# dmosopt/dmosopt

Hardware: NVIDIA H100
Metric: candidate-evals/sec (GP+sort+HV) pop=65536 dim=30 obj=3 (higher is better)
Workload: dtype f64 results; GP variance contraction in split-fp16 wgmma with fp32 accumulation (precision=auto: calibrated against the float64 path, 0 of 65535 rows of the last step recomputed in float64); ranks on u32 ids

## Files before the change

dmosopt_b200/csrc/common.cuh:

```cuda
#pragma once

#include <cuda_runtime.h>
#include <math.h>
#include <stdint.h>
#include <stdio.h>

#include <string>
#include <vector>

#include "../../include/dmosopt_b200.h"

struct dmo_ctx {
  int device = 0;
  cudaStream_t stream = nullptr;
  cudaMemPool_t pool = nullptr;
  cudaEvent_t ev0 = nullptr, ev1 = nullptr;
  int sm_count = 132;
  int64_t launches = 0;
  int64_t waits = 0;
  std::string err;
  void* flush_buf = nullptr;
  size_t flush_bytes = 0;
  int* dev_flag = nullptr;
  uint64_t h2d_bytes = 0, d2h_bytes = 0;
  unsigned long long* lag_host = nullptr;
  cudaEvent_t lag_ev[3] = {nullptr, nullptr, nullptr};
  static constexpr int kSide = 4;
  cudaStream_t side[kSide] = {};
  cudaEvent_t side_ev[kSide + 1] = {};
  bool profiling = false;
  struct Timer {
    std::string name;
    cudaEvent_t a, b;
  };
  std::vector<Timer> timers;
};

struct ProfileScope {
  dmo_ctx* ctx;
  int idx = -1;
  ProfileScope(dmo_ctx* c, const char* name) : ctx(c) {
    if (!c->profiling) return;
    dmo_ctx::Timer t;
    t.name = name;
    if (cudaEventCreate(&t.a) != cudaSuccess || cudaEventCreate(&t.b) != cudaSuccess) return;
    cudaEventRecord(t.a, c->stream);
    c->timers.push_back(t);
    idx = (int)c->timers.size() - 1;
  }
  ~ProfileScope() {
    if (idx >= 0) cudaEventRecord(ctx->timers[idx].b, ctx->stream);
  }
};

int dmo_fail(dmo_ctx* ctx, int code, const char* fmt, ...);

#define DMO_CUDA(call)                                                                        \
  do {                                                                                        \
    cudaError_t e__ = (call);                                                                 \
    if (e__ != cudaSuccess)                                                                   \
      return dmo_fail(ctx, DMO_ERR_CUDA, "%s failed: %s (%s:%d)", #call, cudaGetErrorString(e__), \
                      __FILE__, __LINE__);                                                    \
  } while (0)

#define DMO_TRY(expr)              \
  do {                             \
    int s__ = (expr);              \
    if (s__ != DMO_OK) return s__; \
  } while (0)

#define DMO_REQUIRE(cond, ...)                                 \
  do {                                                         \
    if (!(cond)) return dmo_fail(ctx, DMO_ERR_ARG, __VA_ARGS__); \
  } while (0)

#define DMO_LAUNCH(kernel, grid, block, smem, ...)                       \
  do {                                                                   \
    kernel<<<(grid), (block), (smem), ctx->stream>>>(__VA_ARGS__);       \
    ctx->launches++;                                                     \
  } while (0)

#define DMO_CHECK_LAUNCH() DMO_CUDA(cudaGetLastError())

struct SideStreams {
  dmo_ctx* ctx;
  cudaStream_t main;
  int k = 0;
  int rc = DMO_OK;
  SideStreams(dmo_ctx* c, int nside);
  ~SideStreams();
  void on(int s) { ctx->stream = ctx->side[s]; }
  void back() { ctx->stream = main; }
};

int dmo_lag_slots(dmo_ctx* ctx);

static inline cudaError_t dmo_wait(dmo_ctx* ctx) {
  ctx->waits++;
  return cudaStreamSynchronize(ctx->stream);
}

static inline int64_t ceil_div(int64_t a, int64_t b) { return (a + b - 1) / b; }

template <typename T>
struct DevBuf {
  dmo_ctx* ctx = nullptr;
  T* p = nullptr;
  size_t n = 0;
  DevBuf() {}
  DevBuf(const DevBuf&) = delete;
  DevBuf& operator=(const DevBuf&) = delete;
  ~DevBuf() { release(); }
  int alloc(dmo_ctx* c, size_t count) {
    release();
    ctx = c;
    n = count;
    if (count == 0) count = 1;
    cudaError_t e = cudaMallocAsync((void**)&p, count * sizeof(T), c->stream);
    if (e != cudaSuccess) {
      p = nullptr;
      return dmo_fail(c, DMO_ERR_CUDA, "cudaMallocAsync(%zu bytes) failed: %s", count * sizeof(T),
                      cudaGetErrorString(e));
    }
    return DMO_OK;
  }
  void release() {
    if (p) cudaFreeAsync(p, ctx->stream);
    p = nullptr;
  }
};

bool dmo_is_device_ptr(const void* p);

template <typename T>
struct In {
  DevBuf<T> buf;
  const T* d = nullptr;
  int init(dmo_ctx* ctx, const T* src, size_t count) {
    if (src == nullptr || count == 0) {
      d = nullptr;
      return DMO_OK;
    }
    if (dmo_is_device_ptr(src)) {
      d = src;
      return DMO_OK;
    }
    DMO_TRY(buf.alloc(ctx, count));
    DMO_CUDA(cudaMemcpyAsync(buf.p, src, count * sizeof(T), cudaMemcpyHostToDevice, ctx->stream));
    ctx->h2d_bytes += count * sizeof(T);
    d = buf.p;
    return DMO_OK;
  }
};

template <typename T>
struct Out {
  DevBuf<T> buf;
  T* d = nullptr;
  T* host = nullptr;
  size_t count = 0;
  int init(dmo_ctx* ctx, T* dst, size_t cnt) {
    count = cnt;
    if (dst == nullptr) {
      d = nullptr;
      return DMO_OK;
    }
    if (dmo_is_device_ptr(dst)) {
      d = dst;
      return DMO_OK;
    }
    host = dst;
    DMO_TRY(buf.alloc(ctx, cnt));
    d = buf.p;
    return DMO_OK;
  }
  int finish(dmo_ctx* ctx, size_t cnt = (size_t)-1) {
    if (host && d) {
      size_t c = (cnt == (size_t)-1) ? count : cnt;
// ... 118 lines not shown
```

dmosopt_b200/csrc/ctx.cu:

```cuda
#include <stdarg.h>

#include "common.cuh"

int dmo_fail(dmo_ctx* ctx, int code, const char* fmt, ...) {
  char buf[1024];
  va_list ap;
  va_start(ap, fmt);
  vsnprintf(buf, sizeof(buf), fmt, ap);
  va_end(ap);
  if (ctx) ctx->err = buf;
  return code;
}

bool dmo_is_device_ptr(const void* p) {
  cudaPointerAttributes a;
  cudaError_t e = cudaPointerGetAttributes(&a, p);
  if (e != cudaSuccess) {
    cudaGetLastError();
    return false;
  }
  return a.type == cudaMemoryTypeDevice || a.type == cudaMemoryTypeManaged;
}

int dmo_lag_slots(dmo_ctx* ctx) {
  if (ctx->lag_host) return DMO_OK;
  DMO_CUDA(cudaHostAlloc((void**)&ctx->lag_host, 3 * sizeof(unsigned long long), cudaHostAllocDefault));
  for (cudaEvent_t& e : ctx->lag_ev) DMO_CUDA(cudaEventCreateWithFlags(&e, cudaEventDisableTiming));
  return DMO_OK;
}

SideStreams::SideStreams(dmo_ctx* c, int nside) : ctx(c), main(c->stream) {
  if (nside > dmo_ctx::kSide) nside = dmo_ctx::kSide;
  if (!ctx->side[0]) {
    for (cudaStream_t& st : ctx->side)
      if (cudaStreamCreateWithFlags(&st, cudaStreamNonBlocking) != cudaSuccess) rc = DMO_ERR_CUDA;
    for (cudaEvent_t& e : ctx->side_ev)
      if (cudaEventCreateWithFlags(&e, cudaEventDisableTiming) != cudaSuccess) rc = DMO_ERR_CUDA;
  }
  if (rc == DMO_OK && cudaEventRecord(ctx->side_ev[0], main) != cudaSuccess) rc = DMO_ERR_CUDA;
  for (int s = 0; rc == DMO_OK && s < nside; ++s, ++k)
    if (cudaStreamWaitEvent(ctx->side[s], ctx->side_ev[0], 0) != cudaSuccess) rc = DMO_ERR_CUDA;
  if (rc != DMO_OK) dmo_fail(ctx, rc, "could not set up side streams");
}

SideStreams::~SideStreams() {
  ctx->stream = main;
  for (int s = 0; s < k; ++s) {
    cudaEventRecord(ctx->side_ev[1 + s], ctx->side[s]);
    cudaStreamWaitEvent(main, ctx->side_ev[1 + s], 0);
  }
}

extern "C" {

int dmo_version(void) { return 100; }

int dmo_create(int device, dmo_ctx** out) {
  if (!out) return DMO_ERR_ARG;
  *out = nullptr;
  dmo_ctx* ctx = new dmo_ctx();
  ctx->device = device;
  cudaError_t e = cudaSetDevice(device);
  if (e != cudaSuccess) {
    fprintf(stderr, "dmosopt_b200: cudaSetDevice(%d) failed: %s\n", device, cudaGetErrorString(e));
    delete ctx;
    return DMO_ERR_CUDA;
  }
  cudaDeviceProp prop;
  e = cudaGetDeviceProperties(&prop, device);
  if (e != cudaSuccess) {
    delete ctx;
    return DMO_ERR_CUDA;
  }
  ctx->sm_count = prop.multiProcessorCount;
  if (cudaStreamCreateWithFlags(&ctx->stream, cudaStreamNonBlocking) != cudaSuccess ||
      cudaEventCreate(&ctx->ev0) != cudaSuccess || cudaEventCreate(&ctx->ev1) != cudaSuccess) {
    delete ctx;
    return DMO_ERR_CUDA;
  }
  if (cudaDeviceGetDefaultMemPool(&ctx->pool, device) == cudaSuccess) {
    uint64_t thr = UINT64_MAX;
    cudaMemPoolSetAttribute(ctx->pool, cudaMemPoolAttrReleaseThreshold, &thr);
  }
  if (cudaMalloc((void**)&ctx->dev_flag, 4 * sizeof(int)) != cudaSuccess) {
    delete ctx;
    return DMO_ERR_CUDA;
  }
  cudaMemset(ctx->dev_flag, 0, 4 * sizeof(int));
  *out = ctx;
  return DMO_OK;
}

int dmo_destroy(dmo_ctx* ctx) {
  if (!ctx) return DMO_OK;
  cudaSetDevice(ctx->device);
  dmo_wait(ctx);
  if (ctx->flush_buf) cudaFree(ctx->flush_buf);
  if (ctx->dev_flag) cudaFree(ctx->dev_flag);
  if (ctx->lag_host) cudaFreeHost(ctx->lag_host);
  for (cudaEvent_t e : ctx->lag_ev)
    if (e) cudaEventDestroy(e);
  for (cudaEvent_t e : ctx->side_ev)
    if (e) cudaEventDestroy(e);
  for (cudaStream_t st : ctx->side)
    if (st) cudaStreamDestroy(st);
  cudaEventDestroy(ctx->ev0);
  cudaEventDestroy(ctx->ev1);
  cudaStreamDestroy(ctx->stream);
  delete ctx;
  return DMO_OK;
}

const char* dmo_last_error(dmo_ctx* ctx) { return ctx ? ctx->err.c_str() : "null context"; }

int dmo_synchronize(dmo_ctx* ctx) {
  DMO_CUDA(dmo_wait(ctx));
  return DMO_OK;
}

void* dmo_stream(dmo_ctx* ctx) { return (void*)ctx->stream; }
int64_t dmo_launch_count(dmo_ctx* ctx) { return ctx->launches; }
int64_t dmo_wait_count(dmo_ctx* ctx) { return ctx->waits; }
int dmo_sm_count(dmo_ctx* ctx) { return ctx->sm_count; }

int dmo_timer_begin(dmo_ctx* ctx) {
  DMO_CUDA(cudaEventRecord(ctx->ev0, ctx->stream));
  return DMO_OK;
}

int dmo_timer_end(dmo_ctx* ctx, float* ms) {
  DMO_CUDA(cudaEventRecord(ctx->ev1, ctx->stream));
  ctx->waits++;
  DMO_CUDA(cudaEventSynchronize(ctx->ev1));
  DMO_CUDA(cudaEventElapsedTime(ms, ctx->ev0, ctx->ev1));
  return DMO_OK;
}

int dmo_host_alloc(void** out, uint64_t bytes) {
  return cudaHostAlloc(out, bytes ? bytes : 1, cudaHostAllocDefault) == cudaSuccess ? DMO_OK : DMO_ERR_CUDA;
}
int dmo_host_free(void* p) { return cudaFreeHost(p) == cudaSuccess ? DMO_OK : DMO_ERR_CUDA; }

int dmo_device_alloc(dmo_ctx* ctx, void** out, uint64_t bytes) {
  if (!ctx || !out) return DMO_ERR_ARG;
  DMO_CUDA(cudaSetDevice(ctx->device));
  DMO_CUDA(cudaMallocAsync(out, bytes ? bytes : 1, ctx->stream));
  return DMO_OK;
}
int dmo_device_free(dmo_ctx* ctx, void* p) {
  if (!ctx) return DMO_ERR_ARG;
  if (!p) return DMO_OK;
  DMO_CUDA(cudaFreeAsync(p, ctx->stream));
  return DMO_OK;
}

int dmo_memcpy(dmo_ctx* ctx, void* dst, const void* src, uint64_t bytes) {
  if (!ctx) return DMO_ERR_ARG;
  if (bytes == 0) return DMO_OK;
  DMO_CUDA(cudaMemcpyAsync(dst, src, bytes, cudaMemcpyDefault, ctx->stream));
  DMO_CUDA(dmo_wait(ctx));
  const bool sd = dmo_is_device_ptr(src), dd = dmo_is_device_ptr(dst);
  if (!sd && dd) ctx->h2d_bytes += bytes;
  if (sd && !dd) ctx->d2h_bytes += bytes;
  return DMO_OK;
}

int dmo_transfer_bytes(dmo_ctx* ctx, uint64_t* h2d, uint64_t* d2h) {
  if (h2d) *h2d = ctx->h2d_bytes;
  if (d2h) *d2h = ctx->d2h_bytes;
  return DMO_OK;
}

int dmo_profile_enable(dmo_ctx* ctx, int on) {
  DMO_CUDA(dmo_wait(ctx));
  for (auto& t : ctx->timers) {
    cudaEventDestroy(t.a);
    cudaEventDestroy(t.b);
  }
  ctx->timers.clear();
  ctx->profiling = on != 0;
  return DMO_OK;
}

int dmo_profile_report(dmo_ctx* ctx, char* buf, uint64_t cap) {
  DMO_CUDA(dmo_wait(ctx));
  std::vector<std::string> names;
  std::vector<double> ms;
  std::vector<int> cnt;
// ... 48 lines not shown
```

dmosopt_b200/csrc/gp.cu:

```cuda
#include <string.h>

#include <algorithm>

#include "gp.cuh"

namespace {

constexpr int TRI_B = 128;

__global__ void tri_embed_kernel(const double* __restrict__ L, int64_t ldl, int64_t sL, int64_t N, int64_t Np,
                                 double* __restrict__ Lp) {
  int64_t t = (int64_t)blockIdx.x * blockDim.x + threadIdx.x;
  if (t >= Np * Np) return;
  L += (size_t)blockIdx.y * sL;
  Lp += (size_t)blockIdx.y * Np * Np;
  int64_t r = t / Np, c = t - r * Np;
  Lp[t] = (r < N && c < N) ? (c <= r ? L[r * ldl + c] : 0.0) : (r == c ? 1.0 : 0.0);
}

__global__ void __launch_bounds__(TRI_B) tri_diag_inverse_kernel(const double* __restrict__ Lp, int64_t Np,
                                                                 double* __restrict__ X) {
  Lp += (size_t)blockIdx.y * Np * Np;
  X += (size_t)blockIdx.y * Np * Np;
  const int64_t base = (int64_t)blockIdx.x * TRI_B;
// ... 459 lines not shown
  if (t >= n * M) return;
  const int64_t r = t / M;
  const int m = (int)(t - r * M);
  const int64_t p = idx[r];
  mean[p * M + m] = msub[t];
  var[p * M + m] = vsub[t];
}

int gp_calibrate(dmo_ctx* ctx, dmo_gp* gp) {
  if (gp->calibrated) return DMO_OK;
  const int M = gp->M, d = gp->d;
  const int P = CAL_PROBES;
  gp->auto_mean_tensor = gp->auto_var_tensor = gp->auto_mean_only = false;
  gp->cal_mean_err = gp->cal_var_err = gp->cal_mean_err_only = INFINITY;
  gp->refine_theta = 1.0;
  if (M > 16 || d > 64) {
    gp->calibrated = true;
    return DMO_OK;
  }
  DevBuf<double> xn, m64, v64, mt, vt;
  DMO_TRY(xn.alloc(ctx, (size_t)P * d));
  DMO_TRY(m64.alloc(ctx, (size_t)P * M));
  DMO_TRY(v64.alloc(ctx, (size_t)P * M));
  DMO_TRY(mt.alloc(ctx, (size_t)P * M));
  DMO_TRY(vt.alloc(ctx, (size_t)P * M));
  DMO_LAUNCH(probe_points_kernel, (unsigned)ceil_div(P, 128), 128, 0, gp->Xt.p, gp->N, d, P / 2, P, xn.p);
  DMO_CHECK_LAUNCH();
  const bool prof = ctx->profiling;
  ctx->profiling = false;
  DevBuf<double> mo;
  DMO_TRY(mo.alloc(ctx, (size_t)P * M));
  int rc = gp_predict_fp64(ctx, gp, xn.p, P, m64.p, v64.p);
  if (rc == DMO_OK) rc = gp_predict_tensor(ctx, gp, xn.p, P, mt.p, vt.p);
  if (rc == DMO_OK) rc = gp_predict_tensor(ctx, gp, xn.p, P, mo.p, nullptr);
  ctx->profiling = prof;
  if (rc != DMO_OK) return rc;
  std::vector<double> h((size_t)4 * P * M), ho((size_t)P * M);
  DMO_CUDA(cudaMemcpyAsync(ho.data(), mo.p, (size_t)P * M * 8, cudaMemcpyDeviceToHost, ctx->stream));
  DMO_CUDA(cudaMemcpyAsync(h.data(), m64.p, (size_t)P * M * 8, cudaMemcpyDeviceToHost, ctx->stream));
  DMO_CUDA(cudaMemcpyAsync(h.data() + (size_t)P * M, v64.p, (size_t)P * M * 8, cudaMemcpyDeviceToHost, ctx->stream));
  DMO_CUDA(cudaMemcpyAsync(h.data() + (size_t)2 * P * M, mt.p, (size_t)P * M * 8, cudaMemcpyDeviceToHost, ctx->stream));
  DMO_CUDA(cudaMemcpyAsync(h.data() + (size_t)3 * P * M, vt.p, (size_t)P * M * 8, cudaMemcpyDeviceToHost, ctx->stream));
  DMO_CUDA(dmo_wait(ctx));
  const double *a64 = h.data(), *b64 = a64 + (size_t)P * M, *at = b64 + (size_t)P * M, *bt = at + (size_t)P * M;
  double em = 0.0, ev = 0.0, eo = 0.0;
  for (int p = 0; p < P; ++p)
    for (int m = 0; m < M; ++m) {
      const double ys = gp->h_ystd[m];
      const double prior = (gp->h_constant[m] + gp->h_noise[m]) * ys * ys;
      const double dm = fabs(at[p * M + m] - a64[p * M + m]) / fmax(fabs(a64[p * M + m]), ys);
      const double dv = fabs(bt[p * M + m] - b64[p * M + m]) / prior;
      em = (dm > em || dm != dm) ? (dm != dm ? INFINITY : dm) : em;
      ev = (dv > ev || dv != dv) ? (dv != dv ? INFINITY : dv) : ev;
      const double dq = fabs(ho[p * M + m] - a64[p * M + m]) / fmax(fabs(a64[p * M + m]), ys);
      eo = (dq > eo || dq != dq) ? (dq != dq ? INFINITY : dq) : eo;
    }
  gp->cal_mean_err = em;
  gp->cal_mean_err_only = eo;
  gp->cal_var_err = ev;
  gp->auto_mean_tensor = em <= 2.5e-6;
  gp->auto_mean_only = eo <= 2.5e-6;
  gp->auto_var_tensor = gp->auto_mean_tensor && ev <= 4.5e-6;
  gp->refine_theta = fmax(0.02, 2.0 * ev / 1e-5);
  gp->calibrated = true;
  if (getenv("DMO_GP_VERBOSE"))
    fprintf(stderr, "dmosopt_b200: GP calibration (N=%lld d=%d M=%d): mean err K*alpha %.3e, mean-only kernel %.3e, var err/prior %.3e -> mean %s, var %s, theta %.3f\n",
            (long long)gp->N, d, M, em, eo, ev, gp->auto_mean_tensor ? "K*alpha pass" : "float64", gp->auto_var_tensor ? "tensor" : "float64", gp->refine_theta);
  return DMO_OK;
}

int gp_predict_auto(dmo_ctx* ctx, dmo_gp* gp, const double* dXn, int64_t P, double* d_mean, double* d_var,
                    GpPending* pending) {
  DMO_TRY(gp_calibrate(ctx, gp));
  gp->last_refined = 0;
  if (d_var ? !gp->auto_var_tensor : !gp->auto_mean_only) {
    gp->last_refined = P;
    return gp_predict_fp64(ctx, gp, dXn, P, d_mean, d_var);
  }
  if (!d_var) return gp_predict_tensor(ctx, gp, dXn, P, d_mean, nullptr);
  GpPending own;
  GpPending& q = pending ? *pending : own;
  DMO_TRY(q.flag.alloc(ctx, (size_t)P + 1));
  DMO_TRY(q.pos.alloc(ctx, (size_t)P + 2));
  DMO_TRY(gp_predict_tensor(ctx, gp, dXn, P, d_mean, d_var, q.pos.p + P + 1));
  DMO_CUDA(cudaMemsetAsync(q.flag.p + P, 0, sizeof(int32_t), ctx->stream));
  DMO_LAUNCH(flag_small_var_kernel, (unsigned)ceil_div(P, 256), 256, 0, d_var, P, gp->M, gp->constant.p, gp->noise.p, gp->ystd.p,
             gp->refine_theta, q.flag.p);
  DMO_TRY(prim_exclusive_sum_i32(ctx, q.flag.p, q.pos.p, P + 1));
  DMO_TRY(dmo_lag_slots(ctx));
  DMO_CUDA(cudaMemcpyAsync(ctx->lag_host + 2, q.pos.p + P, 2 * sizeof(int32_t), cudaMemcpyDeviceToHost, ctx->stream));
  DMO_CUDA(cudaEventRecord(ctx->lag_ev[2], ctx->stream));
  q.active = true;
  q.P = P;
  q.dXn = dXn;
  q.d_mean = d_mean;
  q.d_var = d_var;
  if (pending) return DMO_OK;
  bool refined = false;
  return gp_predict_finish(ctx, gp, q, &refined);
}

}

__global__ void linear_mean_add_kernel(const double* __restrict__ Xn, int64_t P, int d, int M,
                                       const double* __restrict__ w, const double* __restrict__ b,
                                       const double* __restrict__ ystd, double* __restrict__ mean) {
  const int64_t t = (int64_t)blockIdx.x * blockDim.x + threadIdx.x;
  if (t >= P * M) return;
  const int64_t p = t / M;
  const int m = (int)(t - p * M);
  double s = b[m];
  for (int j = 0; j < d; ++j) s = fma(w[m * d + j], Xn[p * d + j], s);
  mean[t] += ystd[m] * s;
}

int gp_predict_finish(dmo_ctx* ctx, dmo_gp* gp, GpPending& q, bool* refined) {
  *refined = false;
  if (!q.active) return DMO_OK;
  q.active = false;
  ctx->waits++;
  DMO_CUDA(cudaEventSynchronize(ctx->lag_ev[2]));
  int32_t h[2];
  memcpy(h, ctx->lag_host + 2, sizeof(h));
  if (h[1]) return dmo_fail(ctx, DMO_ERR_INTERNAL, "%s", GP_WATCHDOG_MSG);
  const int32_t n_ref = h[0];
  gp->last_refined = n_ref;
  if (n_ref == 0) return DMO_OK;
  const int M = gp->M, d = gp->d;
  const int64_t P = q.P;
  DevBuf<int32_t> idx;
  DevBuf<double> xs, ms, vs;
  DMO_TRY(idx.alloc(ctx, (size_t)n_ref));
  DMO_TRY(xs.alloc(ctx, (size_t)n_ref * d));
  DMO_TRY(ms.alloc(ctx, (size_t)n_ref * M));
  DMO_TRY(vs.alloc(ctx, (size_t)n_ref * M));
  DMO_LAUNCH(compact_rows_kernel, (unsigned)ceil_div(P, 256), 256, 0, q.flag.p, q.pos.p, P, d, q.dXn, idx.p, xs.p);
  {
    ProfileScope ps(ctx, "gp_refine_fp64");
    DMO_TRY(gp_predict_fp64(ctx, gp, xs.p, n_ref, ms.p, vs.p));
  }
  DMO_LAUNCH(scatter_rows_kernel, (unsigned)ceil_div((int64_t)n_ref * M, 256), 256, 0, idx.p, (int64_t)n_ref, M, ms.p, vs.p,
             q.d_mean, q.d_var);
  DMO_CHECK_LAUNCH();
  *refined = true;
  return DMO_OK;
}

int gp_predict_device(dmo_ctx* ctx, dmo_gp* gp, const double* dX, int64_t P, double* d_mean, double* d_var, int precision,
                      GpPending* pending) {
  const bool defer = pending && precision == DMO_GP_AUTO && d_var && !gp->has_linear_mean;
  DevBuf<double> own;
  DevBuf<double>& xn = defer ? pending->xn : own;
  DMO_TRY(xn.alloc(ctx, (size_t)P * gp->d));
  DMO_LAUNCH(normalise_x_kernel, (unsigned)ceil_div(P * gp->d, 256), 256, 0, dX, P, gp->d, gp->xlb.p, gp->xrg.p, xn.p);
  if (precision == DMO_GP_FP64) {
    DMO_TRY(gp_predict_fp64(ctx, gp, xn.p, P, d_mean, d_var));
  } else if (precision == DMO_GP_TENSOR) {
    DMO_TRY(gp_predict_tensor(ctx, gp, xn.p, P, d_mean, d_var));
  } else if (precision == DMO_GP_AUTO) {
    DMO_TRY(gp_predict_auto(ctx, gp, xn.p, P, d_mean, d_var, defer ? pending : nullptr));
  } else {
    return dmo_fail(ctx, DMO_ERR_ARG, "gp_predict: unknown precision %d", precision);
  }
  if (gp->has_linear_mean) {
    DMO_LAUNCH(linear_mean_add_kernel, (unsigned)ceil_div(P * gp->M, 256), 256, 0, xn.p, P, gp->d, gp->M, gp->lin_w.p,
               gp->lin_b.p, gp->ystd.p, d_mean);
    DMO_CHECK_LAUNCH();
// ... 209 lines not shown
```

dmosopt_b200/csrc/gp.cuh:

```cuda
#pragma once
#include <vector>

#include "common.cuh"

struct GpVarOps {
  int64_t Npad = 0;
  int G = 0;
  std::vector<double> h_kscale;
  DevBuf<double> Linv;
  bool tensor_ready = false;
  DevBuf<uint16_t> Lhi, Llo;
  DevBuf<float> Lscale;
  DevBuf<int> Kexp;
  int alloc(dmo_ctx* ctx, int64_t N, int G);
};

struct dmo_gp {
  int64_t N = 0;
  int d = 0, M = 0, kernel = 0;
  bool isotropic = true;
  GpVarOps ops;
  std::vector<int> h_cov, h_lead;
  DevBuf<int> cov;
  DevBuf<double> Xt;
  DevBuf<double> alpha;
  DevBuf<double> inv_ls;
  DevBuf<double> g_inv_ls, g_constant;
  DevBuf<double> constant, noise, ymean, ystd;
  DevBuf<double> xlb, xrg;
  std::vector<double> h_constant, h_noise, h_ystd;
  bool has_linear_mean = false;
  DevBuf<double> lin_w, lin_b;
  DevBuf<float> Xtf;
  DevBuf<float> CAf;
  bool calibrated = false;
  bool auto_mean_tensor = false;
  bool auto_var_tensor = false;
  double cal_mean_err = 0.0;
  bool auto_mean_only = false;
  double cal_mean_err_only = 0.0;
  double cal_var_err = 0.0;
  double refine_theta = 1.0;
  int64_t last_refined = 0;
};

__device__ __forceinline__ double stationary(double s2, int kind) {
  if (kind == DMO_KERNEL_MATERN52) {
    const double K = sqrt(s2) * 2.23606797749978969641;
    return (1.0 + K + K * K / 3.0) * exp(-K);
  }
  return exp(-0.5 * s2);
}

constexpr int64_t GP_MAX_CHUNK = (int64_t)1 << 20;

int gp_predict_fp64(dmo_ctx* ctx, dmo_gp* gp, const double* dXn, int64_t P, double* d_mean, double* d_var);

int gp_linv_from_factor(dmo_ctx* ctx, const double* L, int64_t N, int64_t ldo, double* dst);
int gp_linv_from_factor_batched(dmo_ctx* ctx, const double* L, int64_t ldl, int64_t sL, int64_t N, int nbat, int64_t ldo,
                                int64_t sdst, double* dst);
int gp_fit_batched(dmo_ctx* ctx, int64_t N, int d, int nbat, int kernel, const double* X, const double* inv_ls, const double* constant,
                   const double* diag_add, const double* y, double* A, int64_t ld, int* info, double* work, double* alpha, double* lml);
int gp_potrf_batched(dmo_ctx* ctx, double* A, int64_t ld, int nbat, int* info);
constexpr int GP_F64_TILE = 128;
int gp_var_contract_fp64(dmo_ctx* ctx, const GpVarOps& ops, const double* Ks, int64_t kplane, int64_t Pcpad, int nsplit,
                         double* vnorm, int64_t vn_ld);
int gp_prepare_tensor(dmo_ctx* ctx, GpVarOps& ops);
constexpr int GP_TC_TILE = 128;
int gp_tensor_var_planes(int64_t Npad);
int gp_var_contract_tensor(dmo_ctx* ctx, const GpVarOps& ops, const uint16_t* Kh, const uint16_t* Kl, int64_t k_alloc,
                           int64_t k_rows, int64_t Pcpad, double* vnorm, int64_t vn_ld, int* abort_flag);
int gp_predict_tensor(dmo_ctx* ctx, dmo_gp* gp, const double* dXn, int64_t P, double* d_mean, double* d_var,
                      int* abort_flag = nullptr);
extern const char* const GP_WATCHDOG_MSG;
struct GpPending {
  bool active = false;
  int64_t P = 0;
  const double* dXn = nullptr;
  double *d_mean = nullptr, *d_var = nullptr;
  DevBuf<double> xn;
  DevBuf<int32_t> flag, pos;
};
int gp_predict_device(dmo_ctx* ctx, dmo_gp* gp, const double* dX, int64_t P, double* d_mean, double* d_var, int precision,
                      GpPending* pending = nullptr);
int gp_predict_finish(dmo_ctx* ctx, dmo_gp* gp, GpPending& pending, bool* refined);

struct GpUnitPredict {
  const char* who = "";
  bool tensor = false;
  int64_t tile = 0;
  int64_t Pc_alloc = 0;
  int n_vp = 0;
  DevBuf<double> vnorm, Ks;
  DevBuf<uint16_t> Kh, Kl;
  DevBuf<int> abort_flag;
  int check(dmo_ctx* ctx, const char* who, int precision, int d);
  int alloc(dmo_ctx* ctx, int64_t P, int64_t Npad, int planes, bool want_var);
  int contract(dmo_ctx* ctx, const GpVarOps& ops, int64_t Pcpad);
  int watchdog(dmo_ctx* ctx);
};

template <typename T>
int upload(dmo_ctx* ctx, DevBuf<T>& dst, const std::vector<T>& src) {
  DMO_TRY(dst.alloc(ctx, src.size()));
  DMO_CUDA(cudaMemcpyAsync(dst.p, src.data(), src.size() * sizeof(T), cudaMemcpyHostToDevice, ctx->stream));
  return DMO_OK;
}

int sv_gemm(dmo_ctx* ctx, int64_t m, int64_t n, int64_t K, double alpha, const double* A, int64_t sai, int64_t sak, const double* B,
            int64_t sbk, int64_t sbj, double diag, double* C, int64_t ldc);
int sv_flip(dmo_ctx* ctx, const double* C, int64_t n, double s, double* O, int64_t ldo);
int svgp_latent_moments(dmo_ctx* ctx, dmo_svgp* sv, GpUnitPredict& up, const double* X, int64_t P, double* fm, double* fv);
struct SvLatentView {
  const double *O0, *O1, *A, *XtT, *inv_ls;
  int64_t Npad;
};
int svgp_latent_view(const dmo_svgp* sv, int l, SvLatentView* v);

constexpr int MT_MAX = 8;
constexpr int MT_FIT_DMAX = 90;
struct MtBlocks {
  std::vector<double> hx, ls, hB, hD, hw, hb;
  std::vector<double> sqD, lam, Q;
  std::vector<double> xs;
  std::vector<double> blk_lml;
  double lml = 0.0;
  DevBuf<double> Lf;
};
int mtgp_blocks_fit(dmo_ctx* ctx, const char* who, int64_t N, int d, int M, const double* X_train, const double* Y,
                    const double* length_scale, const double* B, const double* D, const double* weight, const double* bias,
                    MtBlocks& mb, double* alpha_out);

int mt_scale_inputs(dmo_ctx* ctx, const double* X, int64_t P, int d, const double* xlb, const double* xrg, const double* inv_ls,
                    double* xs);
int64_t mt_kstar_span(bool tensor);
template <typename F>
std::vector<double> mt_xt_transposed(int64_t N, int d, int64_t Npad, F x) {
  std::vector<double> xtT((size_t)d * Npad, 0.0);
  for (int64_t n = 0; n < N; ++n)
    for (int k = 0; k < d; ++k) xtT[(size_t)k * Npad + n] = x(n, k);
  return xtT;
}
int mt_kstar_produce(dmo_ctx* ctx, bool tensor, const double* xs, int64_t P, int64_t p_base, int64_t Pcpad, const double* XtT, int64_t N,
                     int64_t Npad, int d, int M, const double* A, const int* k_exp, double* Ks, uint16_t* Kh, uint16_t* Kl,
                     double* mpart, int64_t mp_ld);
```

dmosopt_b200/csrc/gp_tensor.cu:

```cuda
#include <cuda.h>
#include <cuda_fp16.h>
#include <cudaTypedefs.h>
#include <stdlib.h>

#include "gp.cuh"

namespace {

constexpr int TN = 256;
constexpr int TMV = 128;
constexpr int TK = 32;
constexpr int UK = 16;
constexpr int STAGES = 4;
constexpr int A_BYTES = TMV * TK * 2;
constexpr int B_BYTES = TN * TK * 2;
constexpr int STAGE_BYTES = 2 * A_BYTES + 2 * B_BYTES;
constexpr size_t GEMM_SMEM = (size_t)STAGES * STAGE_BYTES + 1024 + 256;
constexpr int NTHREADS = 384;

__device__ __forceinline__ uint32_t smem_u32(const void* p) { return (uint32_t)__cvta_generic_to_shared(p); }

__device__ __forceinline__ void mbar_init(uint64_t* bar, uint32_t count) {
  asm volatile("mbarrier.init.shared::cta.b64 [%0], %1;" ::"r"(smem_u32(bar)), "r"(count) : "memory");
}
// ... 816 lines not shown
      *n_per_block = npb;
    }
  }
  return best;
}

int gp_mean_direct(dmo_ctx* ctx, dmo_gp* gp, const double* dXn, int64_t P, double* d_mean) {
  const int64_t N = gp->N, Npad = gp->ops.Npad;
  const int M = gp->M, d = gp->d;
  DMO_TRY(prepare_direct_state(ctx, gp));
  DevBuf<double> mpart;
  for (int64_t p_base = 0; p_base < P; p_base += GP_MAX_CHUNK) {
    const int64_t Pc = (P - p_base) < GP_MAX_CHUNK ? (P - p_base) : GP_MAX_CHUNK;
    const int64_t n_qb = ceil_div(Pc, KM_Q);
    int64_t n_per_block = Npad;
    const int64_t nsplit = pick_slices(n_qb, Npad, KM_NS, (int64_t)4 * ctx->sm_count, &n_per_block);
    const int64_t ld = n_qb * KM_Q;
    DMO_TRY(mpart.alloc(ctx, (size_t)nsplit * M * ld));
    dim3 grid((unsigned)nsplit, (unsigned)n_qb);
    {
      ProfileScope ps_(ctx, "gp_mean_direct");
#define KM_LAUNCH(ISO_, MT_)                                                                                                  \
  do {                                                                                                                      \
    if (d <= 16)                                                                                                            \
      DMO_LAUNCH((gp_mean_direct_kernel<ISO_, MT_, 4>), grid, KM_T, 0, dXn, P, p_base, gp->Xtf.p, N, Npad, n_per_block,     \
                 d, gp->kernel, gp->inv_ls.p, gp->constant.p, gp->alpha.p, mpart.p, ld);                                    \
    else                                                                                                                    \
      DMO_LAUNCH((gp_mean_direct_kernel<ISO_, MT_, 8>), grid, KM_T, 0, dXn, P, p_base, gp->Xtf.p, N, Npad, n_per_block,     \
                 d, gp->kernel, gp->inv_ls.p, gp->constant.p, gp->alpha.p, mpart.p, ld);                                    \
  } while (0)
#define KM_SWITCH(ISO_)        \
  switch (M) {                 \
    case 1: KM_LAUNCH(ISO_, 1); break; \
    case 2: KM_LAUNCH(ISO_, 2); break; \
    case 3: KM_LAUNCH(ISO_, 3); break; \
    case 4: KM_LAUNCH(ISO_, 4); break; \
    case 5: KM_LAUNCH(ISO_, 5); break; \
    default: KM_LAUNCH(ISO_, 6); break; \
  }
      if (gp->isotropic) {
        KM_SWITCH(true)
      } else {
        KM_SWITCH(false)
      }
#undef KM_SWITCH
#undef KM_LAUNCH
    }
    DMO_LAUNCH(mean_finish_tc_kernel, (unsigned)ceil_div(Pc * M, 256), 256, 0, mpart.p, (int)nsplit, Pc, ld, M, gp->ymean.p,
               gp->ystd.p, p_base, d_mean);
  }
  DMO_CHECK_LAUNCH();
  return DMO_OK;
}

}

int gp_prepare_tensor(dmo_ctx* ctx, GpVarOps& ops) {
  if (ops.tensor_ready) return DMO_OK;
  const int G = ops.G;
  const int64_t Npad = ops.Npad;
  std::vector<int> kexp(G);
  for (int g = 0; g < G; ++g) {
    double c = ops.h_kscale[g];
    kexp[g] = (c > 0.0) ? 13 - ilogb(c) : 13;
  }
  DMO_TRY(ops.Kexp.alloc(ctx, G));
  DMO_CUDA(cudaMemcpyAsync(ops.Kexp.p, kexp.data(), G * sizeof(int), cudaMemcpyHostToDevice, ctx->stream));
  DMO_CUDA(dmo_wait(ctx));
  DMO_TRY(ops.Lhi.alloc(ctx, (size_t)G * Npad * Npad));
  DMO_TRY(ops.Llo.alloc(ctx, (size_t)G * Npad * Npad));
  DMO_TRY(ops.Lscale.alloc(ctx, (size_t)G * Npad));
  DMO_LAUNCH(split_linv_kernel, (unsigned)(G * Npad), 256, 0, ops.Linv.p, Npad, ops.Kexp.p, ops.Lhi.p, ops.Llo.p,
             ops.Lscale.p);
  DMO_CHECK_LAUNCH();
  ops.tensor_ready = true;
  return DMO_OK;
}

static_assert(TMV == GP_TC_TILE, "gp.cuh exports the wgmma candidate tile");

int gp_tensor_var_planes(int64_t Npad) { return (int)((Npad / TN + 1) / 2); }

int gp_var_contract_tensor(dmo_ctx* ctx, const GpVarOps& ops, const uint16_t* Kh, const uint16_t* Kl, int64_t k_alloc,
                           int64_t k_rows, int64_t Pcpad, double* vnorm, int64_t vn_ld, int* abort_flag) {
  const int64_t Npad = ops.Npad;
  DMO_REQUIRE(Npad % TN == 0 && Pcpad % TMV == 0, "gp_var_contract_tensor: internal padding error");
  CUtensorMap map_kh, map_kl, map_lh, map_ll;
  DMO_TRY(make_map(ctx, &map_kh, Kh, (uint64_t)k_alloc, (uint64_t)Npad, TMV, TK, CU_TENSOR_MAP_SWIZZLE_64B));
  DMO_TRY(make_map(ctx, &map_kl, Kl, (uint64_t)k_alloc, (uint64_t)Npad, TMV, TK, CU_TENSOR_MAP_SWIZZLE_64B));
  DMO_TRY(make_map(ctx, &map_lh, ops.Lhi.p, (uint64_t)ops.G * Npad, (uint64_t)Npad, TN, TK, CU_TENSOR_MAP_SWIZZLE_64B));
  DMO_TRY(make_map(ctx, &map_ll, ops.Llo.p, (uint64_t)ops.G * Npad, (uint64_t)Npad, TN, TK, CU_TENSOR_MAP_SWIZZLE_64B));
  DMO_CUDA(cudaFuncSetAttribute(gp_var_wgmma_kernel, cudaFuncAttributeMaxDynamicSharedMemorySize, (int)GEMM_SMEM));
  GemmParams prm;
  prm.M = ops.G;
  prm.n_pb = (int)(Pcpad / TMV);
  prm.n_jt = (int)(Npad / TN);
  prm.n_q = gp_tensor_var_planes(Npad);
  prm.k_rows = k_rows;
  prm.l_rows = Npad;
  prm.inv_scale = ops.Lscale.p;
  prm.vnorm = vnorm;
  prm.vn_ld = vn_ld;
  prm.abort_flag = abort_flag;
  const int n_work = prm.M * prm.n_pb * prm.n_q;
  const int grid = n_work < ctx->sm_count ? n_work : ctx->sm_count;
  DMO_LAUNCH(gp_var_wgmma_kernel, grid, NTHREADS, GEMM_SMEM, map_kh, map_kl, map_lh, map_ll, prm);
  return DMO_OK;
}

const char* const GP_WATCHDOG_MSG = "gp_predict(tensor): pipeline watchdog tripped (mbarrier wait timed out)";

int gp_predict_tensor(dmo_ctx* ctx, dmo_gp* gp, const double* dXn, int64_t P, double* d_mean, double* d_var, int* abort_flag) {
  const int64_t N = gp->N, Npad = gp->ops.Npad;
  const int M = gp->M, G = gp->ops.G, d = gp->d;
  DMO_REQUIRE(M <= 16, "gp_predict(tensor): at most 16 objectives per model (got %d)", M);
  DMO_REQUIRE(d <= 64, "gp_predict(tensor): at most 64 input dimensions (got %d); use DMO_GP_FP64", d);
  DMO_REQUIRE(Npad % TN == 0, "gp_predict(tensor): internal padding error");
  if (!d_var && d <= KM_D && M <= 6)
    return gp_mean_direct(ctx, gp, dXn, P, d_mean);
  DMO_TRY(gp_prepare_tensor(ctx, gp->ops));
  constexpr int64_t TMv = KM_Q;
  int64_t Pc_max = ((int64_t)6 << 30) / ((int64_t)G * Npad * 4);
  if (Pc_max > GP_MAX_CHUNK) Pc_max = GP_MAX_CHUNK;
  Pc_max = (Pc_max / TMv) * TMv;
  if (Pc_max < TMv) Pc_max = TMv;
  const int64_t Pc_alloc = P < Pc_max ? ceil_div(P, TMv) * TMv : Pc_max;
  const int n_q = gp_tensor_var_planes(Npad);
  DevBuf<uint16_t> Kh, Kl;
  DevBuf<double> vnorm;
  DevBuf<int> own_flag;
  DMO_TRY(Kh.alloc(ctx, (size_t)G * Pc_alloc * Npad));
  DMO_TRY(Kl.alloc(ctx, (size_t)G * Pc_alloc * Npad));
  DMO_TRY(vnorm.alloc(ctx, (size_t)n_q * G * Pc_alloc));
  const bool read_back = abort_flag == nullptr;
  if (read_back) {
    DMO_TRY(own_flag.alloc(ctx, 1));
    abort_flag = own_flag.p;
  }
  DMO_CUDA(cudaMemsetAsync(abort_flag, 0, sizeof(int), ctx->stream));
  const int64_t kplane = Pc_alloc * Npad;
  const bool fused = d <= KM_D && M <= 6 && (gp->isotropic || G <= 2) &&
                     !(getenv("DMO_GP_FUSED") && atoi(getenv("DMO_GP_FUSED")) == 0);
  DevBuf<double> mpart;
  if (fused) DMO_TRY(prepare_direct_state(ctx, gp));
  for (int64_t p_base = 0; p_base < P; p_base += Pc_alloc) {
    const int64_t Pc = (P - p_base) < Pc_alloc ? (P - p_base) : Pc_alloc;
    const int64_t Pcpad = ceil_div(Pc, TMv) * TMv;
    if (fused) {
      int64_t n_per_block = Npad;
      const int64_t n_qb = Pcpad / KM_Q;
      const int64_t nsplit = pick_slices(n_qb, Npad, KF_NS, (int64_t)3 * ctx->sm_count, &n_per_block);
      DMO_TRY(mpart.alloc(ctx, (size_t)nsplit * M * Pcpad));
      dim3 gf((unsigned)nsplit, (unsigned)(Pcpad / KS_Q));
      const size_t smem = kstar_mean_smem(M);
      {
        ProfileScope ps_(ctx, "gp_kstar");
#define KF_LAUNCH(ISO_, MT_, GR_)                                                                                          \
  do {                                                                                                                     \
    DMO_CUDA(cudaFuncSetAttribute(kstar_mean_kernel<ISO_, MT_, GR_>, cudaFuncAttributeMaxDynamicSharedMemorySize, (int)smem)); \
    DMO_LAUNCH((kstar_mean_kernel<ISO_, MT_, GR_>), gf, KS_T, smem, dXn, P, p_base, gp->Xtf.p, N, Npad, n_per_block, d,          \
               gp->kernel, G, gp->cov.p, gp->g_inv_ls.p, gp->g_constant.p, gp->ops.Kexp.p, gp->CAf.p, kplane, Kh.p, Kl.p,   \
               mpart.p, Pcpad);                                                                                            \
  } while (0)
#define KF_SWITCH(ISO_)                                         \
  if (G < M) {                                                  \
    switch (M) {                                    \
      case 2: KF_LAUNCH(ISO_, 2, true); break;                  \
      case 3: KF_LAUNCH(ISO_, 3, true); break;                  \
      case 4: KF_LAUNCH(ISO_, 4, true); break;                  \
      case 5: KF_LAUNCH(ISO_, 5, true); break;                  \
      default: KF_LAUNCH(ISO_, 6, true); break;                 \
    }                                                           \
  } else {                                                      \
    switch (M) {                                                \
      case 1: KF_LAUNCH(ISO_, 1, false); break;                 \
      case 2: KF_LAUNCH(ISO_, 2, false); break;                 \
      case 3: KF_LAUNCH(ISO_, 3, false); break;                 \
      case 4: KF_LAUNCH(ISO_, 4, false); break;                 \
      case 5: KF_LAUNCH(ISO_, 5, false); break;                 \
      default: KF_LAUNCH(ISO_, 6, false); break;                \
    }                                                           \
  }
        if (gp->isotropic) {
          KF_SWITCH(true)
        } else {
          KF_SWITCH(false)
        }
#undef KF_SWITCH
#undef KF_LAUNCH
      }
      DMO_LAUNCH(mean_finish_tc_kernel, (unsigned)ceil_div(Pc * M, 256), 256, 0, mpart.p, (int)nsplit, Pc, Pcpad, M, gp->ymean.p,
                 gp->ystd.p, p_base, d_mean);
    } else {
      {
        ProfileScope ps_(ctx, "gp_kstar");
        const int dmax = d <= 32 ? 32 : 64;
        size_t smem = (size_t)(KT_TP * dmax + G * dmax + G) * sizeof(float);
        dim3 gk((unsigned)(Npad / (2 * KT_TN)), (unsigned)ceil_div(Pcpad, KT_TP));
#define KSTAR_LAUNCH(ISO_, DM_)                                                                                          \
  DMO_LAUNCH((kstar_tensor_kernel<ISO_, DM_>), gk, KT_TN, smem, dXn, P, p_base, Pcpad, gp->Xt.p, N, d, G, gp->kernel, \
             gp->g_inv_ls.p, gp->g_constant.p, gp->ops.Kexp.p, Npad, kplane, Kh.p, Kl.p)
        if (gp->isotropic) {
          if (d <= 32)
            KSTAR_LAUNCH(true, 32);
          else
            KSTAR_LAUNCH(true, 64);
        } else {
          if (d <= 32)
            KSTAR_LAUNCH(false, 32);
          else
            KSTAR_LAUNCH(false, 64);
        }
#undef KSTAR_LAUNCH
      }
      {
        ProfileScope ps_(ctx, "gp_mean");
        DMO_LAUNCH(mean_split_kernel, (unsigned)ceil_div(Pc * M * 32, 256), 256, 0, Kh.p, Kl.p, Pc, N, Npad, kplane, M,
                   gp->cov.p, gp->ops.Kexp.p, gp->alpha.p, gp->ymean.p, gp->ystd.p, p_base, d_mean);
      }
    }
    if (d_var) {
      {
        ProfileScope ps_(ctx, "gp_var");
        DMO_TRY(gp_var_contract_tensor(ctx, gp->ops, Kh.p, Kl.p, G * Pc_alloc, Pc_alloc, Pcpad, vnorm.p, Pc_alloc, abort_flag));
      }
      DMO_LAUNCH(var_finish_tc_kernel, (unsigned)ceil_div(Pc * M, 256), 256, 0, vnorm.p, n_q, Pc, Pc_alloc, M, G,
                 gp->cov.p, gp->constant.p, gp->noise.p, gp->ystd.p, p_base, d_var);
    }
  }
  DMO_CHECK_LAUNCH();
  if (!read_back) return DMO_OK;
  int h_abort = 0;
  DMO_CUDA(cudaMemcpyAsync(&h_abort, abort_flag, sizeof(int), cudaMemcpyDeviceToHost, ctx->stream));
  DMO_CUDA(dmo_wait(ctx));
  if (h_abort) return dmo_fail(ctx, DMO_ERR_INTERNAL, "%s", GP_WATCHDOG_MSG);
  return DMO_OK;
}
```

dmosopt_b200/csrc/step.cu:

```cuda
#include <string.h>

#include "common.cuh"
#include "gp.cuh"

extern "C" {
int dmo_nsga2_step(dmo_ctx* ctx, dmo_gp* gp, double* pop_x, double* pop_y, int32_t* rank, int64_t pop, int d, int M,
                   double crossover_prob, double mutation_prob, double mutation_rate, const double* di_crossover,
                   const double* di_mutation, const double* xlb, const double* xub, uint64_t seed, uint64_t stream_id,
                   int precision, int distance_metric, int with_variance, int round_to_f32, const double* hv_ref, int64_t* n_children,
                   double* hv_out) {
  if (!ctx) return DMO_ERR_ARG;
  DMO_CUDA(cudaSetDevice(ctx->device));
  DMO_REQUIRE(gp && pop_x && pop_y && rank && pop >= 2 && d >= 1 && M >= 1 && di_crossover && di_mutation && xlb && xub,
              "nsga2_step: bad arguments");
  DMO_REQUIRE(distance_metric == DMO_METRIC_NONE || distance_metric == DMO_METRIC_CROWDING || distance_metric == DMO_METRIC_EUCLIDEAN,
              "nsga2_step: unknown distance metric %d", distance_metric);
  DMO_REQUIRE(dmo_is_device_ptr(pop_x) && dmo_is_device_ptr(pop_y) && dmo_is_device_ptr(rank),
              "nsga2_step: the population (pop_x, pop_y, rank) must be resident on the device");
  int64_t poolsize = pop / 2;
  if ((pop & 1) && (poolsize & 1)) poolsize += 1;
  const int64_t cap = pop + 1;
  DevBuf<int64_t> pool, perm;
  DevBuf<double> Xs, Ys, var;
  DevBuf<int32_t> kind;
  DMO_TRY(pool.alloc(ctx, poolsize));
  DMO_TRY(perm.alloc(ctx, pop));
  DMO_TRY(Xs.alloc(ctx, (size_t)(cap + pop) * d));
  DMO_TRY(Ys.alloc(ctx, (size_t)(cap + pop) * M));
  DMO_TRY(kind.alloc(ctx, cap));
  if (with_variance) DMO_TRY(var.alloc(ctx, (size_t)cap * M));
  In<double> idc, idm, ilb, iub;
  DMO_TRY(idc.init(ctx, di_crossover, d));
  DMO_TRY(idm.init(ctx, di_mutation, d));
  DMO_TRY(ilb.init(ctx, xlb, d));
  DMO_TRY(iub.init(ctx, xub, d));
  {
    ProfileScope ps(ctx, "step_tournament");
    DMO_TRY(tournament_device(ctx, rank, nullptr, pop, poolsize, seed, stream_id, pool.p, nullptr));
  }
  int64_t P = 0;
  {
    ProfileScope ps(ctx, "step_generate");
    DMO_TRY(nsga2_generate_device(ctx, pop_x, d, pool.p, poolsize, pop, crossover_prob, mutation_prob, mutation_rate, idc.d, idm.d,
                                  ilb.d, iub.d, seed, stream_id + 1, Xs.p, kind.p, &P, nullptr));
  }
  if (n_children) *n_children = P;
  {
    ProfileScope ps(ctx, "step_truncate");
    DMO_CUDA(cudaMemcpyAsync(Xs.p + (size_t)P * d, pop_x, (size_t)pop * d * sizeof(double), cudaMemcpyDeviceToDevice, ctx->stream));
    DMO_CUDA(cudaMemcpyAsync(Ys.p + (size_t)P * M, pop_y, (size_t)pop * M * sizeof(double), cudaMemcpyDeviceToDevice, ctx->stream));
  }
  GpPending gpp;
  DevBuf<int32_t> rank_in;
  if (P > 0) {
    ProfileScope ps(ctx, "step_gp");
    DMO_TRY(gp_predict_device(ctx, gp, Xs.p, P, Ys.p, with_variance ? var.p : nullptr, precision, &gpp));
  }
  if (gpp.active) {
    DMO_TRY(rank_in.alloc(ctx, pop));
    DMO_CUDA(cudaMemcpyAsync(rank_in.p, rank, (size_t)pop * sizeof(int32_t), cudaMemcpyDeviceToDevice, ctx->stream));
  }
  auto truncate = [&]() -> int {
    ProfileScope ps(ctx, "step_truncate");
    DMO_TRY(remove_worst_device(ctx, Xs.p, Ys.p, P + pop, d, M, distance_metric, nullptr, 0, pop, pop_x, pop_y, rank, perm.p));
    if (round_to_f32) DMO_TRY(prim_round_f32(ctx, pop_y, pop * M));
    return DMO_OK;
  };
  DMO_TRY(truncate());
  bool refined = false;
  const int rc = gp_predict_finish(ctx, gp, gpp, &refined);
  if (rc != DMO_OK) {
    DMO_CUDA(cudaMemcpyAsync(pop_x, Xs.p + (size_t)P * d, (size_t)pop * d * sizeof(double), cudaMemcpyDeviceToDevice, ctx->stream));
    DMO_CUDA(cudaMemcpyAsync(pop_y, Ys.p + (size_t)P * M, (size_t)pop * M * sizeof(double), cudaMemcpyDeviceToDevice, ctx->stream));
    DMO_CUDA(cudaMemcpyAsync(rank, rank_in.p, (size_t)pop * sizeof(int32_t), cudaMemcpyDeviceToDevice, ctx->stream));
    DMO_CUDA(dmo_wait(ctx));
    return rc;
  }
  if (refined) DMO_TRY(truncate());
  if (hv_ref && hv_out) {
    ProfileScope ps(ctx, "step_hv");
    DMO_REQUIRE(M <= 16, "nsga2_step: too many objectives for the hypervolume");
    double h_ref[16];
    if (dmo_is_device_ptr(hv_ref)) {
      ctx->waits++;
      DMO_CUDA(cudaMemcpyAsync(h_ref, hv_ref, M * sizeof(double), cudaMemcpyDeviceToHost, ctx->stream));
    } else {
      memcpy(h_ref, hv_ref, M * sizeof(double));
    }
    DMO_TRY(hypervolume_device_ranked(ctx, pop_y, pop, M, h_ref, rank, hv_out));
  }
  return DMO_OK;
}
}
```

Baseline: 8.377 million.

## Overlap first truncation with GP variance contraction on separate streams

Records an event once the GP mean for the last chunk is ready, then runs the first non-dominated sort/truncation on a side lane stream while the variance wgmma contraction runs on a high-priority stream. The variance kernel grid can optionally leave SMs free (DMO_GP_VAR_RESERVE), and the grid sizing now balances work per CTA. This aims to hide the sorting cost behind the tensor-core variance work. The price is extra streams and events and some contention between concurrent kernels.

```diff
diff --git a/dmosopt_b200/csrc/common.cuh b/dmosopt_b200/csrc/common.cuh
--- a/dmosopt_b200/csrc/common.cuh
+++ b/dmosopt_b200/csrc/common.cuh
@@ -28,6 +28,8 @@
   static constexpr int kSide = 4;
   cudaStream_t side[kSide] = {};
   cudaEvent_t side_ev[kSide + 1] = {};
+  cudaStream_t lane = nullptr, gp_hi = nullptr;
+  cudaEvent_t lane_ev[4] = {};
   bool profiling = false;
   struct Timer {
     std::string name;
@@ -94,6 +96,7 @@
 };
 
 int dmo_lag_slots(dmo_ctx* ctx);
+int dmo_lane_streams(dmo_ctx* ctx);
 
 static inline cudaError_t dmo_wait(dmo_ctx* ctx) {
   ctx->waits++;
diff --git a/dmosopt_b200/csrc/ctx.cu b/dmosopt_b200/csrc/ctx.cu
--- a/dmosopt_b200/csrc/ctx.cu
+++ b/dmosopt_b200/csrc/ctx.cu
@@ -26,6 +26,17 @@
   if (ctx->lag_host) return DMO_OK;
   DMO_CUDA(cudaHostAlloc((void**)&ctx->lag_host, 3 * sizeof(unsigned long long), cudaHostAllocDefault));
   for (cudaEvent_t& e : ctx->lag_ev) DMO_CUDA(cudaEventCreateWithFlags(&e, cudaEventDisableTiming));
+  return DMO_OK;
+}
+
+int dmo_lane_streams(dmo_ctx* ctx) {
+  if (ctx->gp_hi) return DMO_OK;
+  int least = 0, greatest = 0;
+  DMO_CUDA(cudaDeviceGetStreamPriorityRange(&least, &greatest));
+  for (cudaEvent_t& e : ctx->lane_ev)
+    if (!e) DMO_CUDA(cudaEventCreateWithFlags(&e, cudaEventDisableTiming));
+  if (!ctx->lane) DMO_CUDA(cudaStreamCreateWithFlags(&ctx->lane, cudaStreamNonBlocking));
+  DMO_CUDA(cudaStreamCreateWithPriority(&ctx->gp_hi, cudaStreamNonBlocking, greatest));
   return DMO_OK;
 }
 
@@ -104,6 +115,10 @@
     if (e) cudaEventDestroy(e);
   for (cudaStream_t st : ctx->side)
     if (st) cudaStreamDestroy(st);
+  for (cudaEvent_t e : ctx->lane_ev)
+    if (e) cudaEventDestroy(e);
+  if (ctx->lane) cudaStreamDestroy(ctx->lane);
+  if (ctx->gp_hi) cudaStreamDestroy(ctx->gp_hi);
   cudaEventDestroy(ctx->ev0);
   cudaEventDestroy(ctx->ev1);
   cudaStreamDestroy(ctx->stream);
diff --git a/dmosopt_b200/csrc/gp.cu b/dmosopt_b200/csrc/gp.cu
--- a/dmosopt_b200/csrc/gp.cu
+++ b/dmosopt_b200/csrc/gp.cu
@@ -565,7 +565,7 @@
   GpPending& q = pending ? *pending : own;
   DMO_TRY(q.flag.alloc(ctx, (size_t)P + 1));
   DMO_TRY(q.pos.alloc(ctx, (size_t)P + 2));
-  DMO_TRY(gp_predict_tensor(ctx, gp, dXn, P, d_mean, d_var, q.pos.p + P + 1));
+  DMO_TRY(gp_predict_tensor(ctx, gp, dXn, P, d_mean, d_var, q.pos.p + P + 1, q.ov.mean_ready ? &q.ov : nullptr));
   DMO_CUDA(cudaMemsetAsync(q.flag.p + P, 0, sizeof(int32_t), ctx->stream));
   DMO_LAUNCH(flag_small_var_kernel, (unsigned)ceil_div(P, 256), 256, 0, d_var, P, gp->M, gp->constant.p, gp->noise.p, gp->ystd.p,
              gp->refine_theta, q.flag.p);
diff --git a/dmosopt_b200/csrc/gp.cuh b/dmosopt_b200/csrc/gp.cuh
--- a/dmosopt_b200/csrc/gp.cuh
+++ b/dmosopt_b200/csrc/gp.cuh
@@ -69,11 +69,16 @@
 constexpr int GP_TC_TILE = 128;
 int gp_tensor_var_planes(int64_t Npad);
 int gp_var_contract_tensor(dmo_ctx* ctx, const GpVarOps& ops, const uint16_t* Kh, const uint16_t* Kl, int64_t k_alloc,
-                           int64_t k_rows, int64_t Pcpad, double* vnorm, int64_t vn_ld, int* abort_flag);
+                           int64_t k_rows, int64_t Pcpad, double* vnorm, int64_t vn_ld, int* abort_flag, int reserve = 0);
+struct GpOverlap {
+  cudaEvent_t mean_ready = nullptr;
+  int reserve = 0;
+};
 int gp_predict_tensor(dmo_ctx* ctx, dmo_gp* gp, const double* dXn, int64_t P, double* d_mean, double* d_var,
-                      int* abort_flag = nullptr);
+                      int* abort_flag = nullptr, const GpOverlap* ov = nullptr);
 extern const char* const GP_WATCHDOG_MSG;
 struct GpPending {
+  GpOverlap ov;
   bool active = false;
   int64_t P = 0;
   const double* dXn = nullptr;
diff --git a/dmosopt_b200/csrc/gp_tensor.cu b/dmosopt_b200/csrc/gp_tensor.cu
--- a/dmosopt_b200/csrc/gp_tensor.cu
+++ b/dmosopt_b200/csrc/gp_tensor.cu
@@ -922,7 +922,7 @@
 int gp_tensor_var_planes(int64_t Npad) { return (int)((Npad / TN + 1) / 2); }
 
 int gp_var_contract_tensor(dmo_ctx* ctx, const GpVarOps& ops, const uint16_t* Kh, const uint16_t* Kl, int64_t k_alloc,
-                           int64_t k_rows, int64_t Pcpad, double* vnorm, int64_t vn_ld, int* abort_flag) {
+                           int64_t k_rows, int64_t Pcpad, double* vnorm, int64_t vn_ld, int* abort_flag, int reserve) {
   const int64_t Npad = ops.Npad;
   DMO_REQUIRE(Npad % TN == 0 && Pcpad % TMV == 0, "gp_var_contract_tensor: internal padding error");
   CUtensorMap map_kh, map_kl, map_lh, map_ll;
@@ -943,14 +943,20 @@
   prm.vn_ld = vn_ld;
   prm.abort_flag = abort_flag;
   const int n_work = prm.M * prm.n_pb * prm.n_q;
-  const int grid = n_work < ctx->sm_count ? n_work : ctx->sm_count;
+  int per_cta = (int)ceil_div(n_work, ctx->sm_count);
+  int grid = (int)ceil_div(n_work, per_cta);
+  if (reserve > 0) {
+    per_cta = (int)ceil_div(n_work, reserve < grid ? grid - reserve : 1);
+    grid = (int)ceil_div(n_work, per_cta);
+  }
   DMO_LAUNCH(gp_var_wgmma_kernel, grid, NTHREADS, GEMM_SMEM, map_kh, map_kl, map_lh, map_ll, prm);
   return DMO_OK;
 }
 
 const char* const GP_WATCHDOG_MSG = "gp_predict(tensor): pipeline watchdog tripped (mbarrier wait timed out)";
 
-int gp_predict_tensor(dmo_ctx* ctx, dmo_gp* gp, const double* dXn, int64_t P, double* d_mean, double* d_var, int* abort_flag) {
+int gp_predict_tensor(dmo_ctx* ctx, dmo_gp* gp, const double* dXn, int64_t P, double* d_mean, double* d_var, int* abort_flag,
+                      const GpOverlap* ov) {
   const int64_t N = gp->N, Npad = gp->ops.Npad;
   const int M = gp->M, G = gp->ops.G, d = gp->d;
   DMO_REQUIRE(M <= 16, "gp_predict(tensor): at most 16 objectives per model (got %d)", M);
@@ -1059,10 +1065,24 @@
                    gp->cov.p, gp->ops.Kexp.p, gp->alpha.p, gp->ymean.p, gp->ystd.p, p_base, d_mean);
       }
     }
+    if (ov && p_base + Pc_alloc >= P) DMO_CUDA(cudaEventRecord(ov->mean_ready, ctx->stream));
     if (d_var) {
       {
         ProfileScope ps_(ctx, "gp_var");
-        DMO_TRY(gp_var_contract_tensor(ctx, gp->ops, Kh.p, Kl.p, G * Pc_alloc, Pc_alloc, Pcpad, vnorm.p, Pc_alloc, abort_flag));
+        cudaStream_t main = ctx->stream;
+        if (ov) {
+          DMO_CUDA(cudaEventRecord(ctx->lane_ev[1], main));
+          DMO_CUDA(cudaStreamWaitEvent(ctx->gp_hi, ctx->lane_ev[1], 0));
+          ctx->stream = ctx->gp_hi;
+        }
+        const int rc = gp_var_contract_tensor(ctx, gp->ops, Kh.p, Kl.p, G * Pc_alloc, Pc_alloc, Pcpad, vnorm.p, Pc_alloc, abort_flag,
+                                              ov ? ov->reserve : 0);
+        if (ov) {
+          ctx->stream = main;
+          DMO_CUDA(cudaEventRecord(ctx->lane_ev[2], ctx->gp_hi));
+          DMO_CUDA(cudaStreamWaitEvent(main, ctx->lane_ev[2], 0));
+        }
+        DMO_TRY(rc);
       }
       DMO_LAUNCH(var_finish_tc_kernel, (unsigned)ceil_div(Pc * M, 256), 256, 0, vnorm.p, n_q, Pc, Pc_alloc, M, G,
                  gp->cov.p, gp->constant.p, gp->noise.p, gp->ystd.p, p_base, d_var);
diff --git a/dmosopt_b200/csrc/step.cu b/dmosopt_b200/csrc/step.cu
--- a/dmosopt_b200/csrc/step.cu
+++ b/dmosopt_b200/csrc/step.cu
@@ -1,3 +1,4 @@
+#include <stdlib.h>
 #include <string.h>
 
 #include "common.cuh"
@@ -50,15 +51,22 @@
     DMO_CUDA(cudaMemcpyAsync(Xs.p + (size_t)P * d, pop_x, (size_t)pop * d * sizeof(double), cudaMemcpyDeviceToDevice, ctx->stream));
     DMO_CUDA(cudaMemcpyAsync(Ys.p + (size_t)P * M, pop_y, (size_t)pop * M * sizeof(double), cudaMemcpyDeviceToDevice, ctx->stream));
   }
+  const char* ov_env = getenv("DMO_STEP_OVERLAP");
+  const bool overlap = !(ov_env && atoi(ov_env) == 0);
+  int var_reserve = 0;
+  if (const char* e = getenv("DMO_GP_VAR_RESERVE")) var_reserve = atoi(e);
+  DMO_REQUIRE(var_reserve >= 0, "nsga2_step: DMO_GP_VAR_RESERVE must not be negative");
   GpPending gpp;
   DevBuf<int32_t> rank_in;
   if (P > 0) {
+    DMO_TRY(rank_in.alloc(ctx, pop));
+    if (overlap) {
+      DMO_TRY(dmo_lane_streams(ctx));
+      gpp.ov.mean_ready = ctx->lane_ev[0];
+      gpp.ov.reserve = var_reserve;
+    }
     ProfileScope ps(ctx, "step_gp");
     DMO_TRY(gp_predict_device(ctx, gp, Xs.p, P, Ys.p, with_variance ? var.p : nullptr, precision, &gpp));
-  }
-  if (gpp.active) {
-    DMO_TRY(rank_in.alloc(ctx, pop));
-    DMO_CUDA(cudaMemcpyAsync(rank_in.p, rank, (size_t)pop * sizeof(int32_t), cudaMemcpyDeviceToDevice, ctx->stream));
   }
   auto truncate = [&]() -> int {
     ProfileScope ps(ctx, "step_truncate");
@@ -66,7 +74,22 @@
     if (round_to_f32) DMO_TRY(prim_round_f32(ctx, pop_y, pop * M));
     return DMO_OK;
   };
-  DMO_TRY(truncate());
+  auto first_truncate = [&]() -> int {
+    if (gpp.active) DMO_CUDA(cudaMemcpyAsync(rank_in.p, rank, (size_t)pop * sizeof(int32_t), cudaMemcpyDeviceToDevice, ctx->stream));
+    return truncate();
+  };
+  if (gpp.active && gpp.ov.mean_ready) {
+    cudaStream_t main = ctx->stream;
+    DMO_CUDA(cudaStreamWaitEvent(ctx->lane, gpp.ov.mean_ready, 0));
+    ctx->stream = ctx->lane;
+    const int rc = first_truncate();
+    ctx->stream = main;
+    DMO_CUDA(cudaEventRecord(ctx->lane_ev[3], ctx->lane));
+    DMO_CUDA(cudaStreamWaitEvent(main, ctx->lane_ev[3], 0));
+    DMO_TRY(rc);
+  } else {
+    DMO_TRY(first_truncate());
+  }
   bool refined = false;
   const int rc = gp_predict_finish(ctx, gp, gpp, &refined);
   if (rc != DMO_OK) {
```

Result: faster. 8.916 million (median of 6 runs) (+6.4%).
